# composewell/streamly-lz4

Hardware: AMD Instinct MI355X
Metric: GB/s uncompressed (compress+decompress), 64 KiB blocks, 1/2/4/8 GPU (higher is better)
Workload: dtype u8

## Files before the change

### streamly-lz4_amd/csrc/decode_par.hpp

```cpp
#pragma once

#include "decode_seq.hpp"

namespace lz4dev {

#define PAR_NODES 512
#ifndef PAR_ADAPT
#define PAR_ADAPT 1
#endif
#ifndef PAR_TAIL_ROUND
#define PAR_TAIL_ROUND 2
#endif
#ifndef PAR_ADAPT6
#define PAR_ADAPT6 416
#endif
#ifndef PAR_ADAPT10
#define PAR_ADAPT10 0
#endif
#define PAR_MAXNODES (PAR_ADAPT10 ? 640 : 512)
#ifndef PAR_SQ
#define PAR_SQ 3
#endif
#ifndef PAR_WIN
#define PAR_WIN 832
#endif
#ifndef PAR_RING
#define PAR_RING 5728
#endif
#ifndef PAR_HIST
#define PAR_HIST 2000
#endif
#ifndef PAR_BATCH_OUT
#define PAR_BATCH_OUT 2048
#endif
#ifndef PAR_FAR_WIDE
#define PAR_FAR_WIDE 0
#endif
#ifndef PAR_RANK
#define PAR_RANK 1
#endif
#ifndef PAR_PRIO
#define PAR_PRIO 0x33
#endif
#ifndef PAR_WAVES
#define PAR_WAVES 5
#endif

struct __attribute__((aligned(16))) ParLds {
    uint8_t win[PAR_WIN + 32];
    uint16_t jump[PAR_MAXNODES + 8];
    uint8_t ring[PAR_RING + 32];
};
#define PAR_END (2 * PAR_NODES)
#ifndef PAR_LDS_LIMIT
#define PAR_LDS_LIMIT 7680
#endif
static_assert(sizeof(ParLds) <= PAR_LDS_LIMIT, "ParLds above six 1280-byte LDS granules: 18 waves per CU instead of 20");
#define PAR_WIN_LANES (PAR_WIN / 16)
static_assert(PAR_WIN % 16 == 0 && PAR_WIN_LANES <= LZ4_WAVE, "the window is 16 bytes per lane");
static_assert(PAR_MAXNODES + 288 <= PAR_WIN + 32, "a plain sequence that starts at the last node, and the reads behind it, stay in win[]");
static_assert(PAR_HIST + 30 + PAR_BATCH_OUT + 32 <= PAR_RING, "a batch fits the ring right after a slide");

typedef uint64_t par_u64u __attribute__((aligned(1)));
typedef uint32_t par_u32u __attribute__((aligned(1)));
typedef uint16_t par_u16u __attribute__((aligned(1)));

typedef uint32_t par_v4 __attribute__((ext_vector_type(4)));
typedef par_v4 par_v4u __attribute__((aligned(1)));

__device__ __forceinline__ uint32_t lds_u32_any(const uint8_t *base4, uint32_t addr)
{
    const uint32_t *p = (const uint32_t *)(base4 + (addr & ~3u));
    return __builtin_amdgcn_alignbyte(p[1], p[0], addr & 3u);
}
__device__ __forceinline__ uint64_t lds_u64_any(const uint8_t *base4, uint32_t addr)
{
    const uint32_t *p = (const uint32_t *)(base4 + (addr & ~3u));
    const uint32_t d0 = p[0], d1 = p[1], d2 = p[2];
    const uint32_t sh = addr & 3u;
    return ((uint64_t)__builtin_amdgcn_alignbyte(d2, d1, sh) << 32) | __builtin_amdgcn_alignbyte(d1, d0, sh);
}

__device__ __forceinline__ int par_bperm(int v, int srcLane)
{
    return __builtin_amdgcn_ds_bpermute(srcLane << 2, v);
}

template <int D>
__device__ __forceinline__ int par_row_shr(int v)
{
    return __builtin_amdgcn_update_dpp(0, v, 0x110 | D, 0xf, 0xf, true);
}

__device__ __forceinline__ int par_scan_incl(int x)
{
    x += __builtin_amdgcn_update_dpp(0, x, 0x111, 0xf, 0xf, true);
    x += __builtin_amdgcn_update_dpp(0, x, 0x112, 0xf, 0xf, true);
    x += __builtin_amdgcn_update_dpp(0, x, 0x114, 0xf, 0xf, true);
    x += __builtin_amdgcn_update_dpp(0, x, 0x118, 0xf, 0xf, true);
    x += __builtin_amdgcn_update_dpp(0, x, 0x142, 0xa, 0xf, false);
    x += __builtin_amdgcn_update_dpp(0, x, 0x143, 0xc, 0xf, false);
    return x;
}

enum { PS_BATCHES, PS_SEQS, PS_ROUNDS, PS_MATCH_ITERS, PS_LIT_ITERS, PS_HANDOVERS, PS_SLIDES, PS_FULL, PS_FAR,
       PS_T_WINDOW, PS_T_SPEC, PS_T_CHAIN, PS_T_DECODE, PS_T_LIT, PS_T_NEED, PS_T_MATCH, PS_T_FLUSH, PS_T_SEQ, PS_COUNT };

template <bool STATS, bool DICT, bool TOL = false, bool LIST = false, bool PARTIAL = false>
__device__ int decode_block_par(const uint8_t *src, int srcLen, uint8_t *dst, int cap, const uint8_t *dict,
                                uint32_t dictLen, const uint8_t *bufLo, const uint8_t *bufHi, ParLds &L,
                                unsigned long long *stats, TolCtx *tol = nullptr, const uint8_t *list = nullptr,
                                int listLen = 0)
{
    int li = 0;
    int nodesPerLane = 8;
    uint32_t sc[PS_COUNT];
    uint32_t tmark = 0;
    if (STATS) {
#pragma unroll
        for (int i = 0; i < PS_COUNT; i++) sc[i] = 0;
        tmark = (uint32_t)__builtin_amdgcn_readfirstlane((int)(uint32_t)__builtin_amdgcn_s_memtime());
    }
    auto lap = [&](int which) {
        if (STATS) {
            const uint32_t now = (uint32_t)__builtin_amdgcn_readfirstlane((int)(uint32_t)__builtin_amdgcn_s_memtime());
            sc[which] += now - tmark;
            tmark = now;
        }
    };
    auto publish = [&]() {
        if (STATS && lane_id() == 0) {
#pragma unroll
            for (int i = 0; i < PS_COUNT; i++) atomicAdd(&stats[i], (unsigned long long)sc[i]);
        }
    };
    static_assert(!PARTIAL || (!DICT && !TOL), "the partial mode has no dictionary");
    if (cap < 128 || srcLen < 64) return decode_block_seq<TOL, PARTIAL>(src, srcLen, dst, cap, dict, dictLen, bufLo, bufHi, tol);
    if (!DICT) { dict = nullptr; dictLen = 0; }
    const uint8_t *dictEnd = DICT ? dict + dictLen : dst;
    const int dictLo = DICT ? -(int)min(dictLen, 65535u) : 0;

    int lane = lane_id();
    const int iend = srcLen;
    const uint32_t A = (uint32_t)((uintptr_t)dst & 15);
    int ip = 0, op = 0;
    int ringBase = 0;
    int flushed = 0;
    SeqState st;

    auto win_lane = [&]() -> int { return (PAR_WIN_LANES < LZ4_WAVE) ? min(lane, PAR_WIN_LANES - 1) : lane; };
    auto fetch_window = [&](uintptr_t base) -> uint4 {
        const uint8_t *q = (const uint8_t *)(base + 16u * (uint32_t)win_lane());
        if (q >= bufLo && q + 16 <= bufHi) {
            const par_v4 v = *as_global((const par_v4 *)q);
            return make_uint4(v.x, v.y, v.z, v.w);
        }
        uint32_t w[4] = {0, 0, 0, 0};
        for (int k = 0; k < 16; k++)
            if (q + k >= bufLo && q + k < bufHi) w[k >> 2] |= (uint32_t)as_global(q)[k] << (8 * (k & 3));
        return make_uint4(w[0], w[1], w[2], w[3]);
    };

#ifndef PAR_FLUSH
#define PAR_FLUSH 64
#endif
    const uint32_t AF = (uint32_t)((uintptr_t)dst & (PAR_FLUSH - 1));
    auto flush = [&](int upto, bool final) {
        wave_fence();
        int f = flushed;
        const int mis = (int)((AF + (uint32_t)f) & (PAR_FLUSH - 1));
        if (mis) {
            const int head = PAR_FLUSH - mis;
            if (upto - f >= head) {
                if (lane < head) dst[f + lane] = L.ring[f - ringBase + (int)A + lane];
                f += head;
            } else if (!final) {
                return;
            }
        }
        if (((AF + (uint32_t)f) & (PAR_FLUSH - 1)) == 0) {
            const int n16 = final ? (upto - f) >> 4 : ((upto - f) / PAR_FLUSH) * (PAR_FLUSH / 16);
            for (int c = lane; c < n16; c += LZ4_WAVE) {
                const uint4 v = *(const uint4 *)&L.ring[f - ringBase + (int)A + 16 * c];
                *(uint4 *)(dst + f + 16 * c) = v;
            }
            f += n16 << 4;
        }
        if (final) {
            for (int x = f + lane; x < upto; x += LZ4_WAVE) dst[x] = L.ring[x - ringBase + (int)A];
            f = upto;
        }
        flushed = f;
        wave_fence();
    };

    uintptr_t wbase = (uintptr_t)src & ~(uintptr_t)15;
    uint4 wnext = fetch_window(wbase);
    bool winStale = true;
    const uint8_t *jumpB = (const uint8_t *)L.jump;

    for (;;) {
        while (iend - ip >= 64 && cap - op >= 128) {
            lap(PS_T_FLUSH);

            const uint8_t *gp = src + ip;
            const uintptr_t abase = (uintptr_t)gp & ~(uintptr_t)15;
            const int wofs = (int)((uintptr_t)gp - abase);
            const int ipW0 = ip - wofs;
            const int iendW = iend - ipW0;
            const int inLim = min(iendW - 32, PAR_WIN);
            if (abase != wbase) { wbase = abase; wnext = fetch_window(abase); winStale = true; }
            if (winStale) {
                *(uint4 *)&L.win[16 * win_lane()] = wnext;
                winStale = false;
                wave_fence();
            }
            lap(PS_T_WINDOW);

            uint32_t c2, absorb;
            bool fromList = false;
            if (LIST && li < listLen) {
                fromList = true;
                absorb = 2u * (uint32_t)max(inLim, 0);
                const int k = li + lane;
                const uint32_t d = (k < listLen) ? (uint32_t)as_global(list)[k] : 0u;
                const uint64_t zm = __ballot(d == 0u);
                const int known = zm ? (int)__builtin_ctzll(zm) : LZ4_WAVE - 1;
                const int incl0 = par_scan_incl((int)d);
                c2 = (lane <= known) ? 2u * (uint32_t)(wofs + incl0 - (int)d) : absorb;
                c2 = min(c2, absorb);
            } else {
            auto parse_square = [&](auto NC) {
                constexpr int NL = decltype(NC)::value;
                static_assert(NL % 2 == 0 && NL * LZ4_WAVE <= PAR_MAXNODES, "pairs of nodes, table size");
                uint32_t J[NL];
                absorb = 2u * ((uint32_t)min(inLim, NL * LZ4_WAVE - 1) + 1u);
                {
                    typedef unsigned short par_h2 __attribute__((ext_vector_type(2)));
                    uint32_t w0, w1, w2;
                    if (NL == 8) {
                        const uint64_t lo = *(const uint64_t *)&L.win[8 * lane];
                        w0 = (uint32_t)lo; w1 = (uint32_t)(lo >> 32);
                        w2 = (uint32_t)__builtin_amdgcn_update_dpp(0, (int)w0, 0x130, 0xf, 0xf, false);
                    } else {
                        const uint32_t a = (uint32_t)(NL * lane);
                        const uint32_t *q = (const uint32_t *)&L.win[a & ~3u];
                        const uint32_t d0 = q[0], d1 = q[1], d2 = q[2], d3 = q[3];
                        const uint32_t sh = a & 3u;
                        w0 = __builtin_amdgcn_alignbyte(d1, d0, sh);
                        w1 = __builtin_amdgcn_alignbyte(d2, d1, sh);
                        w2 = __builtin_amdgcn_alignbyte(d3, d2, sh);
                    }
                    auto h2 = [](uint32_t x) { par_h2 r; __builtin_memcpy(&r, &x, 4); return r; };
                    auto u32 = [](par_h2 x) { uint32_t r; __builtin_memcpy(&r, &x, 4); return r; };
                    const par_h2 one = {1, 1}, lim = h2((absorb >> 1) * 0x00010001u);
                    const uint32_t base3 = ((uint32_t)(NL * lane) + 3u) * 0x00010001u + 0x00010000u;
                    uint32_t P[NL / 2];
#pragma unroll
                    for (int p = 0; p < NL / 2; p++) {
                        const uint32_t ws = (p < 2) ? w0 : ((p < 4) ? w1 : w2), wn = (p < 2) ? w1 : w2;
                        const par_h2 T = h2(__builtin_amdgcn_perm(0u, ws, (p & 1) ? 0x0c030c02u : 0x0c010c00u));
                        const par_h2 B = h2((p & 1) ? __builtin_amdgcn_perm(wn, ws, 0x0c040c03u) : __builtin_amdgcn_perm(0u, ws, 0x0c020c01u));
                        const par_h2 lit0 = T >> 4;
                        const par_h2 ext = (lit0 + one) >> 4;
                        const par_h2 term = ext * (B + one) + lit0;
                        const par_h2 mlx = ((T & (par_h2){15, 15}) + one) >> 4;
                        const par_h2 nxt = term + mlx + h2(base3 + 0x00020002u * (uint32_t)p);
                        P[p] = u32(__builtin_elementwise_min(nxt, lim) << 1);
                    }
                    uint32_t *tw = (uint32_t *)&L.jump[NL * lane];
#pragma unroll
                    for (int p = 0; p < NL / 2; p++) tw[p] = P[p];
                    if (lane == 0) L.jump[NL * LZ4_WAVE] = (uint16_t)(2 * NL * LZ4_WAVE);
#pragma unroll
                    for (int p = 0; p < NL / 2; p++) { J[2 * p] = P[p] & 0xffffu; J[2 * p + 1] = P[p] >> 16; }
                }
                wave_fence();
                lap(PS_T_SPEC);
#if PAR_PRIO
            if ((PAR_PRIO >> 0 & 3) != (PAR_PRIO >> 6 & 3)) __builtin_amdgcn_s_setprio(PAR_PRIO >> 0 & 3);
#endif

                c2 = (lane == 0) ? 2u * (uint32_t)wofs : absorb;
#pragma unroll
                for (int k = 0; k < PAR_SQ; k++) {
                    const int d = 1 << k;
                    const int cj = (int)*(const uint16_t *)(jumpB + c2);
#pragma unroll
                    for (int j = 0; j < NL; j++) J[j] = (uint32_t)*(const uint16_t *)(jumpB + J[j]);
                    int sh;
                    if (k == 0) sh = par_row_shr<1>(cj);
                    else if (k == 1) sh = par_row_shr<2>(cj);
                    else if (k == 2) sh = par_row_shr<4>(cj);
                    else sh = par_row_shr<8>(cj);
                    if (lane >= d && lane < 2 * d) c2 = (uint32_t)sh;
                    wave_fence();
                    uint32_t *tw = (uint32_t *)&L.jump[NL * lane];
#pragma unroll
                    for (int p = 0; p < NL / 2; p++) tw[p] = J[2 * p] | (J[2 * p + 1] << 16);
                    wave_fence();
                }
            };
#ifdef PAR_FORCE_NL
            parse_square(std::integral_constant<int, PAR_FORCE_NL>());
#elif PAR_ADAPT
            if (nodesPerLane == 6) parse_square(std::integral_constant<int, 6>());
#if PAR_ADAPT10
            else if (nodesPerLane == 10) parse_square(std::integral_constant<int, 10>());
#endif
            else
                parse_square(std::integral_constant<int, 8>());
#else
                parse_square(std::integral_constant<int, 8>());
#endif
            {
                constexpr int G = 1 << PAR_SQ;
#pragma unroll
                for (int g = 1; g < LZ4_WAVE / G; g++) {
                    int cj = (int)absorb;
                    if (lane >= G * (g - 1) && lane < G * g) cj = (int)*(const uint16_t *)(jumpB + c2);
                    int sh;
                    if (G == 1 && (g & 15)) sh = par_row_shr<1>(cj);
                    else if (G == 2 && (g & 7)) sh = par_row_shr<2>(cj);
                    else if (G == 4 && (g & 3)) sh = par_row_shr<4>(cj);
                    else if (G == 8 && (g & 1)) sh = par_row_shr<8>(cj);
#ifndef PAR_GROUP_BPERM
                    else if (G == 8 && (g == 2 || g == 6)) {
                        const auto r = __builtin_amdgcn_permlane16_swap((unsigned)cj, (unsigned)cj, false, false);
                        sh = __builtin_amdgcn_update_dpp(0, (int)r[0], 0x128 , 0xf, 0xf, false);
                    } else if (G == 8 && g == 4) {
                        const auto q = __builtin_amdgcn_permlane32_swap((unsigned)cj, (unsigned)cj, false, false);
                        const auto r = __builtin_amdgcn_permlane16_swap(q[0], q[0], false, false);
                        sh = __builtin_amdgcn_update_dpp(0, (int)r[1], 0x128 , 0xf, 0xf, false);
                    }
#endif
                    else sh = par_bperm(cj, (lane - G) & 63);
                    if (lane >= G * g && lane < G * g + G) c2 = (uint32_t)sh;
                }
            }
            }
            lap(PS_T_CHAIN);
#if PAR_PRIO
            if ((PAR_PRIO >> 2 & 3) != (PAR_PRIO >> 0 & 3)) __builtin_amdgcn_s_setprio(PAR_PRIO >> 2 & 3);
#endif

            const bool has = c2 < absorb;
            const uint32_t cc = has ? (c2 >> 1) : 0u;
            const uint32_t tb = lds_u32_any(L.win, cc);
            const uint32_t t = tb & 0xffu, b1 = (tb >> 8) & 0xffu;
            const bool is15 = (t >> 4) == 15u;
            const uint32_t lit = is15 ? 15u + b1 : (t >> 4);
            const uint32_t litStart = cc + 1u + (is15 ? 1u : 0u);
            const uint32_t offPos = litStart + lit;
            const uint32_t ob = lds_u32_any(L.win, offPos);
            const uint32_t off16 = ob & 0xffffu, b2 = (ob >> 16) & 0xffu;
            const bool mlx = (t & 15u) == 15u;
            const uint32_t ml = (t & 15u) + LZ4_MINMATCH + (mlx ? b2 : 0u);
            const uint32_t nxt = offPos + 2u + (mlx ? 1u : 0u);
            bool ok = has && !(is15 && b1 == 255u) && !(mlx && b2 == 255u) && (int)nxt <= inLim && off16 != 0;
            bool listBad = false;
            if (LIST && fromList) {
                const uint32_t prevNxt = (uint32_t)__builtin_amdgcn_update_dpp(0, (int)nxt, 0x138 , 0xf, 0xf, false);
                listBad = has && lane > 0 && prevNxt != cc;
                ok = ok && !listBad;
            }
            const int len = ok ? (int)(lit + ml) : 0;
            const int incl = par_scan_incl(len);
            const int outEnd = op + incl;
            const int outStart = outEnd - len;
            const int dpos = outStart + (int)lit;
            const int spos = dpos - (int)off16;
            ok = ok && incl <= PAR_BATCH_OUT && outEnd + 64 < cap &&
                 ((spos >= 0 && (spos >= ringBase || spos + (int)ml <= flushed)) ||
                  (DICT && spos >= dictLo && spos + (int)ml <= 0 && (!PAR_FAR_WIDE || ml >= 16u || spos + 16 <= 0)) ||
                  (TOL && spos < 0));
            const uint64_t okm = __ballot(ok);
            const int nseq = (~okm) ? (int)__builtin_ctzll(~okm) : LZ4_WAVE;
            if (LIST && fromList) {
                if (nseq < LZ4_WAVE && ((__ballot(listBad) >> nseq) & 1ull)) listLen = 0;
                li += nseq;
            }
            lap(PS_T_DECODE);
            if (STATS) { sc[PS_BATCHES]++; sc[PS_SEQS] += (unsigned)nseq; if (nseq == LZ4_WAVE) sc[PS_FULL]++; }
            if (nseq == 0) break;

            const bool act = lane < nseq;
            const int opNext = __builtin_amdgcn_readlane(outEnd, nseq - 1);
            const int ipNext = ipW0 + __builtin_amdgcn_readlane((int)nxt, nseq - 1);
            if (PAR_ADAPT && !fromList && nseq >= 16) {
                const int need = (ipNext - ip) * LZ4_WAVE;
                nodesPerLane = (need <= PAR_ADAPT6 * nseq) ? 6 : ((need <= 520 * nseq || !PAR_ADAPT10) ? 8 : 10);
            } else if (PAR_ADAPT && !fromList && nodesPerLane == 6 && !((__ballot(has) >> nseq) & 1ull)) {
                nodesPerLane = 8;
            }
            const uint32_t mdA = (uint32_t)(dpos - ringBase) + A;
            const bool ext = TOL && spos < 0;
            const bool nearSrc = spos >= ringBase && !ext;
            bool deferred = false;
            const bool w8 = ml >= 8 && off16 >= 8;
            const bool grp = w8 && (off16 >= 32 || off16 >= ml);
            const bool g16 = grp && ml >= 16;
            const bool g8 = grp && ml < 16;
            const bool g4 = ml < 8 && off16 >= ml;
            const bool fastc = g16 || g8 || g4;

            const uint64_t farm = __ballot(act && !nearSrc);
            if (TOL && farm) {
                if (act && !nearSrc && (ext || tol_tainted(tol, spos, spos + (int)ml))) {
                    deferred = true;
                    tol_taint(tol, dpos, dpos + (int)ml);
                }
                wave_fence();
            }
            const uint8_t *gsrc = (DICT && spos < 0) ? dictEnd + spos : dst + spos;
            const bool farMine = act && !nearSrc && !deferred;
            const uint32_t fstep = (ml >= 16) ? 16u : ((ml >= 8) ? 8u : 4u);
            const uint32_t flast = ml - fstep;
            par_v4 f0 = {0u, 0u, 0u, 0u}, f1 = {0u, 0u, 0u, 0u};
            uint64_t fa = 0, fb = 0;
            uint32_t fw0 = 0, fw1 = 0;
            if (farm) {
                if (STATS) sc[PS_FAR] += (unsigned)__builtin_popcountll(farm);
#if PAR_FAR_WIDE
                if (farMine) __builtin_memcpy(&f0, gsrc, 16);
                if (farMine && fstep == 16 && ml > 16u) __builtin_memcpy(&f1, gsrc + min(16u, flast), 16);
#else
                if (farMine && fstep == 16) {
                    __builtin_memcpy(&f0, gsrc, 16);
                    __builtin_memcpy(&f1, gsrc + min(16u, flast), 16);
                }
                if (farMine && fstep == 8) {
                    fa = *(const par_u64u *)(gsrc);
                    fb = *(const par_u64u *)(gsrc + flast);
                }
                if (farMine && fstep == 4) {
                    fw0 = *(const par_u32u *)(gsrc);
                    fw1 = *(const par_u32u *)(gsrc + flast);
                }
#endif
            }
            {
                const uintptr_t nb = (uintptr_t)(src + ipNext) & ~(uintptr_t)15;
                wbase = nb;
                wnext = fetch_window(nb);
            }

            uint64_t need = 0;
#if PAR_RANK
            {
                static_assert(16 * (PAR_BATCH_OUT / 64 + 1) <= 2 * PAR_NODES, "rank records fit the jump table");
                uint8_t *rk = (uint8_t *)L.jump;
                constexpr int NREC = PAR_BATCH_OUT / 64 + 1;
                {
                    uint32_t z = 0;
                    asm volatile("" : "+v"(z));
                    if (lane < NREC) *(uint4 *)&rk[16 * lane] = make_uint4(z, z, z, z);
                }
                wave_fence();
                if (act) {
                    const uint32_t rel = (uint32_t)(outStart - op);
                    atomicOr((uint32_t *)&rk[16u * (rel >> 6) + 4u * ((rel >> 5) & 1u)], 1u << (rel & 31u));
                }
                wave_fence();
                {
                    uint2 w = make_uint2(0u, 0u);
                    if (lane < NREC) w = *(const uint2 *)&rk[16 * lane];
                    const int cnt = (int)__builtin_popcount(w.x) + (int)__builtin_popcount(w.y);
                    const int pre = par_scan_incl(cnt) - cnt;
                    if (lane < NREC) *(uint32_t *)&rk[16 * lane + 8] = (uint32_t)pre;
                }
                wave_fence();
                const int srcHi = min(spos + (int)ml, outStart);
                if (act && nearSrc && srcHi > op && srcHi > spos) {
                    const uint32_t xlo = (uint32_t)(max(spos, op) - op), xhi = (uint32_t)(srcHi - 1 - op);
                    auto rank = [&](uint32_t x) -> int {
                        const uint4 r = *(const uint4 *)&rk[16u * (x >> 6)];
                        const uint32_t m = (2u << (x & 31u)) - 1u;
                        const bool hi = (x & 32u) != 0u;
                        return (int)r.z + (int)__builtin_popcount(r.x & (hi ? ~0u : m)) + (int)__builtin_popcount(r.y & (hi ? m : 0u)) - 1;
                    };
                    const int jlo = rank(xlo), jhi = rank(xhi);
                    const uint64_t upto = (jhi >= 63) ? ~0ull : ((1ull << (jhi + 1)) - 1ull);
                    need = upto & ~((1ull << jlo) - 1ull);
                    need &= ~(1ull << lane);
                }
                wave_fence();
            }
#else
            {
                const int srcHi = min(spos + (int)ml, outStart);
                const int xlo = max(spos, op), xhi = max(srcHi - 1, op);
                int jlo = 0, jhi = 0;
#pragma unroll
                for (int stp = 32; stp >= 1; stp >>= 1) {
                    const int c1 = jlo + stp, cb = jhi + stp;
                    const int v1 = par_bperm(outStart, c1 & 63), v2 = par_bperm(outStart, cb & 63);
                    if (c1 < nseq && v1 <= xlo) jlo = c1;
                    if (cb < nseq && v2 <= xhi) jhi = cb;
                }
                if (act && nearSrc && srcHi > op && srcHi > spos) {
                    const uint64_t upto = (jhi >= 63) ? ~0ull : ((1ull << (jhi + 1)) - 1ull);
                    need = upto & ~((1ull << jlo) - 1ull);
                    need &= ~(1ull << lane);
                }
            }
#endif
            {
                const uint32_t sA = litStart;
                const uint32_t dA = (uint32_t)(outStart - ringBase) + A;
                const uint32_t n = act ? lit : 0u;
                if (n > 16) {
                    const uint32_t last = n - 16;
                    for (uint32_t o = 0;; o += 16) {
                        const uint32_t oo = min(o, last);
                        *(par_v4u *)&L.ring[dA + oo] = *(const par_v4u *)&L.win[sA + oo];
                        if (o >= last) break;
                    }
                } else if (n > 8) {
                    if (n + ml >= 16) {
                        *(par_v4u *)&L.ring[dA] = *(const par_v4u *)&L.win[sA];
                    } else {
                        const uint64_t a = *(const par_u64u *)&L.win[sA], b = *(const par_u64u *)&L.win[sA + n - 8];
                        *(par_u64u *)&L.ring[dA] = a;
                        *(par_u64u *)&L.ring[dA + n - 8] = b;
                    }
                } else if (n > 0) {
                    const uint64_t v = lds_u64_any(L.win, sA);
                    if (n + ml >= 8) {
                        *(par_u64u *)&L.ring[dA] = v;
                    } else {
                        uint64_t w = v;
                        for (uint32_t q = 0; q < n; q++) { L.ring[dA + q] = (uint8_t)w; w >>= 8; }
                    }
                }
            }
            wave_fence();

            if (farm) {
#if PAR_FAR_WIDE
                if (fstep == 16 && ml <= 16u) f1 = f0;
                {
                    const uint32_t sh = ml - 8u;
                    const bool up = (sh & 4u) != 0u;
                    const uint32_t lo = up ? f0.y : f0.x, mid = up ? f0.z : f0.y, hi = up ? f0.w : f0.z;
                    fa = (uint64_t)f0.x | ((uint64_t)f0.y << 32);
                    fb = (uint64_t)__builtin_amdgcn_alignbyte(mid, lo, sh & 3u) | ((uint64_t)__builtin_amdgcn_alignbyte(hi, mid, sh & 3u) << 32);
                    fw0 = f0.x;
                    fw1 = __builtin_amdgcn_alignbyte(f0.y, f0.x, (ml - 4u) & 3u);
                }
#endif
                if (farMine && fstep == 16) {
                    *(par_v4u *)&L.ring[mdA] = f0;
                    *(par_v4u *)&L.ring[mdA + min(16u, flast)] = f1;
                }
                if (farMine && fstep == 8) {
                    *(par_u64u *)&L.ring[mdA] = fa;
                    *(par_u64u *)&L.ring[mdA + flast] = fb;
                }
                if (farMine && fstep == 4) {
                    *(par_u32u *)&L.ring[mdA] = fw0;
                    *(par_u32u *)&L.ring[mdA + flast] = fw1;
                }
                for (uint32_t base = 32; __ballot(farMine && base < ml); base += 32) {
                    par_v4 v0 = {0u, 0u, 0u, 0u}, v1 = {0u, 0u, 0u, 0u};
                    const bool on = farMine && base < ml;
                    const uint32_t o0 = min(base, flast), o1 = min(base + 16u, flast);
                    if (on) {
                        __builtin_memcpy(&v0, gsrc + o0, 16);
                        __builtin_memcpy(&v1, gsrc + o1, 16);
                    }
                    if (on) {
                        *(par_v4u *)&L.ring[mdA + o0] = v0;
                        *(par_v4u *)&L.ring[mdA + o1] = v1;
                    }
                }
            }

            lap(PS_T_NEED);
#if PAR_PRIO
            if ((PAR_PRIO >> 4 & 3) != (PAR_PRIO >> 2 & 3)) __builtin_amdgcn_s_setprio(PAR_PRIO >> 4 & 3);
#endif
            need &= ~farm;
            uint64_t done = ((nseq >= LZ4_WAVE) ? 0ull : (~0ull << nseq)) | farm;
            bool pending = act && nearSrc;
            const uint32_t msA = nearSrc ? (uint32_t)(spos - ringBase) + A : 0u;
            int roundNo = 0;
            while (~done) {
#if PAR_TAIL_ROUND
                if (!TOL && roundNo >= PAR_TAIL_ROUND) {
                    for (uint64_t sm = __ballot(pending); sm; sm &= sm - 1) {
                        if (STATS) sc[PS_MATCH_ITERS]++;
                        const int k = (int)__builtin_ctzll(sm);
                        const uint32_t kd = (uint32_t)__builtin_amdgcn_readlane((int)mdA, k);
                        const uint32_t ks = (uint32_t)__builtin_amdgcn_readlane((int)msA, k);
                        const uint32_t koff = (uint32_t)__builtin_amdgcn_readlane((int)off16, k);
                        const uint32_t kml = (uint32_t)__builtin_amdgcn_readlane((int)ml, k);
                        if (koff >= kml) {
                            if ((uint32_t)lane < kml) L.ring[kd + (uint32_t)lane] = L.ring[ks + (uint32_t)lane];
                            for (uint32_t j = (uint32_t)lane + LZ4_WAVE; j < kml; j += LZ4_WAVE) L.ring[kd + j] = L.ring[ks + j];
                        } else {
                            const float rcp = 1.0f / (float)koff;
                            for (uint32_t j = (uint32_t)lane; j < kml; j += LZ4_WAVE) {
                                const uint32_t q = (uint32_t)((float)j * rcp);
                                int rem = (int)j - (int)(q * koff);
                                if (rem < 0) rem += (int)koff; else if (rem >= (int)koff) rem -= (int)koff;
                                L.ring[kd + j] = L.ring[ks + (uint32_t)rem];
                            }
                        }
                        wave_fence();
                    }
                    pending = false;
                    break;
                }
                roundNo++;
#endif
                const bool ready = pending && ((need & ~done) == 0ull);
                bool mine = ready;
                if (TOL) {
                    const int srcHi = min(spos + (int)ml, dpos);
                    if (ready && srcHi > spos && tol_tainted(tol, spos, srcHi)) {
                        deferred = true;
                        mine = false;
                        tol_taint(tol, dpos, dpos + (int)ml);
                    }
                    wave_fence();
                }
                if (STATS) sc[PS_ROUNDS]++;
                for (uint32_t base = 0; __ballot(mine && fastc && base < ml); base += 32) {
                    if (STATS) sc[PS_MATCH_ITERS]++;
                    const bool on = mine && fastc && base < ml;
                    const uint32_t cs = g16 ? 16u : (g8 ? 8u : 4u);
                    const uint32_t lastc = ml - cs;
                    const uint32_t o0 = g16 ? min(base, lastc) : 0u;
                    const uint32_t o1 = g16 ? min(base + 16u, lastc) : lastc;
                    par_v4 v0 = {0u, 0u, 0u, 0u}, v1 = {0u, 0u, 0u, 0u};
                    uint64_t na = 0, nc = 0;
                    uint32_t nw0 = 0, nw1 = 0;
                    if (on) v0 = *(const par_v4u *)&L.ring[msA + o0];
                    if (on && g16 && ml > 16u) v1 = *(const par_v4u *)&L.ring[msA + o1];
                    if (g16 && ml <= 16u) v1 = v0;
                    {
                        const uint32_t sh = ml - 8u;
                        const bool up = (sh & 4u) != 0u;
                        const uint32_t lo = up ? v0.y : v0.x, mid = up ? v0.z : v0.y, hi = up ? v0.w : v0.z;
                        na = (uint64_t)v0.x | ((uint64_t)v0.y << 32);
                        nc = (uint64_t)__builtin_amdgcn_alignbyte(mid, lo, sh & 3u) | ((uint64_t)__builtin_amdgcn_alignbyte(hi, mid, sh & 3u) << 32);
                        nw0 = v0.x;
                        nw1 = __builtin_amdgcn_alignbyte(v0.y, v0.x, (ml - 4u) & 3u);
                    }
                    if (on && g16) {
                        *(par_v4u *)&L.ring[mdA + o0] = v0;
                        *(par_v4u *)&L.ring[mdA + o1] = v1;
                    }
                    if (on && g8) {
                        *(par_u64u *)&L.ring[mdA] = na;
                        *(par_u64u *)&L.ring[mdA + o1] = nc;
                    }
                    if (on && g4) {
                        *(par_u32u *)&L.ring[mdA] = nw0;
                        *(par_u32u *)&L.ring[mdA + o1] = nw1;
                    }
                    wave_fence();
                }
                for (uint64_t sm = __ballot(mine && !fastc); sm; sm &= sm - 1) {
                    if (STATS) sc[PS_MATCH_ITERS]++;
                    const int k = (int)__builtin_ctzll(sm);
                    const uint32_t kd = (uint32_t)__builtin_amdgcn_readlane((int)mdA, k);
                    const uint32_t ks = (uint32_t)__builtin_amdgcn_readlane((int)msA, k);
                    const uint32_t koff = (uint32_t)__builtin_amdgcn_readlane((int)off16, k);
                    const uint32_t kml = (uint32_t)__builtin_amdgcn_readlane((int)ml, k);
                    const float rcp = 1.0f / (float)koff;
                    for (uint32_t j = (uint32_t)lane; j < kml; j += LZ4_WAVE) {
                        const uint32_t q = (uint32_t)((float)j * rcp);
                        int rem = (int)j - (int)(q * koff);
                        if (rem < 0) rem += (int)koff; else if (rem >= (int)koff) rem -= (int)koff;
                        L.ring[kd + j] = L.ring[ks + (uint32_t)rem];
                    }
                    wave_fence();
                }
                pending = pending && !ready;
                done |= __ballot(ready);
            }
            wave_fence();
            if (TOL) {
                const uint64_t dm = __ballot(deferred);
                if (dm) {
                    const uint32_t rank = __builtin_amdgcn_mbcnt_hi((uint32_t)(dm >> 32), __builtin_amdgcn_mbcnt_lo((uint32_t)dm, 0u));
                    const uint32_t base = tol->count;
                    if (deferred && base + rank < tol->cap) tol->list[base + rank] = tol_entry(dpos, spos, ml);
                    wave_fence();
                    if (lane == 0) tol->count = base + (uint32_t)__builtin_popcountll(dm);
                    wave_fence();
                }
            }
            lap(PS_T_MATCH);
#if PAR_PRIO
            if ((PAR_PRIO >> 6 & 3) != (PAR_PRIO >> 4 & 3)) __builtin_amdgcn_s_setprio(PAR_PRIO >> 6 & 3);
#endif

            op = opNext;
            ip = ipNext;
            *(uint4 *)&L.win[16 * win_lane()] = wnext;
            wave_fence();
            flush(op, false);
            if (op - ringBase + (int)A + PAR_BATCH_OUT + 32 > PAR_RING) {
                if (STATS) sc[PS_SLIDES]++;
                const int newBase = (op - PAR_HIST) & ~15;
                const int delta = newBase - ringBase;
                const int n16 = (op - newBase + (int)A + 15) >> 4;
                constexpr int PAR_SLIDE = (PAR_HIST + 45 + 16 * LZ4_WAVE - 1) / (16 * LZ4_WAVE);
                {
                    uint4 v[PAR_SLIDE];
#pragma unroll
                    for (int i = 0; i < PAR_SLIDE; i++) {
                        const int k = lane + i * LZ4_WAVE;
                        v[i] = (k < n16) ? *(const uint4 *)&L.ring[delta + 16 * k] : make_uint4(0u, 0u, 0u, 0u);
                    }
                    wave_fence();
#pragma unroll
                    for (int i = 0; i < PAR_SLIDE; i++) {
                        const int k = lane + i * LZ4_WAVE;
                        if (k < n16) *(uint4 *)&L.ring[16 * k] = v[i];
                    }
                }
                ringBase = newBase;
                wave_fence();
            }
        }

        flush(op, true);
        st.ip = ip; st.op = op; st.fast = true;
        const bool tail = (iend - ip < 64 || cap - op < 128);
        if (STATS && !tail) sc[PS_HANDOVERS]++;
        lap(PS_T_FLUSH);
        int r = decode_seq_dispatch<TOL, PARTIAL>(st, tail ? 0 : 1, src, srcLen, dst, cap, dict, dictLen, bufLo, bufHi, tol);
        if (r == SEQ_CONTINUE && (!st.fast || iend - st.ip < 64 || cap - st.op < 128))
            r = decode_seq_dispatch<TOL, PARTIAL>(st, 0, src, srcLen, dst, cap, dict, dictLen, bufLo, bufHi, tol);
        lap(PS_T_SEQ);
        r = uni(r);
        if (r != SEQ_CONTINUE) { publish(); return r; }
        ip = uni(st.ip); op = uni(st.op);
        if (LIST) li += 1;
        asm volatile("v_mbcnt_lo_u32_b32 %0, -1, 0\n\tv_mbcnt_hi_u32_b32 %0, -1, %0" : "=v"(lane));
        wbase = (uintptr_t)(src + ip) & ~(uintptr_t)15;
        wnext = fetch_window(wbase);
        winStale = true;
        wave_fence();
        ringBase = (op > PAR_HIST) ? ((op - PAR_HIST) & ~15) : 0;
        flushed = op;
        for (int x = ringBase + lane; x < op; x += LZ4_WAVE) L.ring[x - ringBase + (int)A] = dst[x];
        wave_fence();
        lap(PS_T_SEQ);
    }
}

}
```

### streamly-lz4_amd/csrc/kernels/decode_par_cu.inc

```
#ifdef PAR_WAVES_MAX
#define PAR_OCC __attribute__((amdgpu_flat_work_group_size(64, 64), amdgpu_waves_per_eu(PAR_WAVES, PAR_WAVES_MAX)))
#else
#define PAR_OCC __launch_bounds__(64, PAR_WAVES)
#endif
template <bool STATS>
__global__ PAR_OCC void k_decode_par(DecodeArgs a, unsigned long long *stats)
{
    __shared__ ParLds lds;
    const int blk = (int)blockIdx.x;
    const uint8_t *data = nullptr;
    int compLen = 0, cap = 0;
    int r = read_block_header(a, blk, data, compLen, cap);
    if (r == 0)
        r = decode_block_par<STATS, false>(data, compLen, a.out + a.outOff[blk], cap, nullptr, 0, a.framed,
                                    a.framed + a.framedLen, lds, stats);
    if (lane_id() == 0) a.result[blk] = r;
}

void launch_decode_par(const DecodeArgs &a, unsigned long long *stats, hipStream_t s)
{
    if (a.nBlocks <= 0) return;
    if (stats)
        hipLaunchKernelGGL(k_decode_par<true>, dim3((unsigned)a.nBlocks), dim3(64), 0, s, a, stats);
    else
        hipLaunchKernelGGL(k_decode_par<false>, dim3((unsigned)a.nBlocks), dim3(64), 0, s, a, stats);
    launch_link_stat(a, s);
}

__global__ PAR_OCC void k_decode_par_redo(DecodeArgs a)
{
    __shared__ ParLds lds;
    const int blk = (int)blockIdx.x;
    if (uni(a.result[blk]) != CU_REDO) return;
    const uint8_t *data = nullptr;
    int compLen = 0, cap = 0;
    int r = read_block_header(a, blk, data, compLen, cap);
    if (r == 0)
        r = decode_block_par<false, false, false, true>(data, compLen, a.out + a.outOff[blk], cap, nullptr, 0, a.framed,
                                                        a.framed + a.framedLen, lds, nullptr, nullptr, nullptr, 0);
    if (lane_id() == 0) a.result[blk] = r;
}

__global__ __launch_bounds__(CU_THREADS) void k_decode_cu(DecodeArgs a)
{
    __shared__ __attribute__((aligned(16))) uint8_t lds[CU_LDS_BYTES];
    const int blk = (int)blockIdx.x;
    const uint8_t *data = nullptr;
    int compLen = 0, cap = 0;
    int r = uni(read_block_header(a, blk, data, compLen, cap));
    if (r == 0 && a.cuBail && (int64_t)uni(compLen) * 16 > (int64_t)uni(cap) * 15) r = CU_REDO;
    else if (r == 0)
        r = decode_block_cu<false>(data, uni(compLen), a.out + a.outOff[blk], uni(cap), nullptr, 0, a.framed, a.framed + a.framedLen, lds,
                                   a.cuDbg ? a.cuDbg + 16 * (size_t)blk : nullptr, a.cuBail != 0);
    if (threadIdx.x == 0) a.result[blk] = r;
    const bool prevFinal = blk == 0 && a.lookBack > 0 && a.cu.res && uni(a.result[-1]) >= 65536;
    if (a.cu.res && (blk > 0 || prevFinal) && r == CU_REDO && !(a.cuBail && (int64_t)uni(compLen) * 16 > (int64_t)uni(cap) * 15)) {
        __syncthreads();
        const uint8_t *dict = prevFinal ? a.out + a.outOff[-1] + (size_t)uni(a.result[-1]) - 65536u : a.run.zeroPage;
        const int r2 = decode_block_cu<true>(data, uni(compLen), a.out + a.outOff[blk], uni(cap), dict, 65536u, a.framed,
                                            a.framed + a.framedLen, lds, nullptr, false, 0);
        if (threadIdx.x == 0) {
            a.cu.res[blk] = r2;
            if (r2 < 0 || (r2 < 65536 && blk + 1 < a.nBlocks)) atomicAdd(&a.cu.flags[1], 1u);
        }
    }
}

__global__ __launch_bounds__(CU_THREADS) void k_decode_cu_linked(DecodeArgs a)
{
    __shared__ __attribute__((aligned(16))) uint8_t lds[CU_LDS_BYTES];
    const int blk = (int)blockIdx.x;
    if (uni(a.result[blk]) >= 0) return;
    const uint8_t *dict = nullptr;
    if (blk == 0) {
        const bool prevFinal = a.lookBack > 0 && uni(a.result[-1]) >= 65536;
        if (prevFinal && uni(a.cu.res[0]) >= 65536) return;
        if (!prevFinal || a.cu.pass != 1) { if (threadIdx.x == 0) atomicAdd(&a.cu.flags[1], 1u); return; }
        dict = a.out + a.outOff[-1] + (size_t)uni(a.result[-1]) - 65536u;
    } else {
        if (a.cu.pass > 2 && uni(a.cu.flags[2 + blk - 1]) == 0u) return;
        dict = a.cu.pass == 1 ? a.run.zeroPage : a.cu.snap + (size_t)(blk - 1) * 65536u;
    }
    const uint8_t *data = nullptr;
    int compLen = 0, cap = 0;
    int r = uni(read_block_header(a, blk, data, compLen, cap));
    if (r == 0)
        r = decode_block_cu<true>(data, uni(compLen), a.out + a.outOff[blk], uni(cap), dict, 65536u, a.framed, a.framed + a.framedLen, lds, nullptr, false,
                                  (blk > 0 && a.cu.pass > 1 && uni(a.cu.res[blk]) >= 65536) ? uni(a.cu.res[blk]) : 0);
    if (threadIdx.x == 0) {
        a.cu.res[blk] = r;
        if (r < 0 || (r < 65536 && blk + 1 < a.nBlocks)) atomicAdd(&a.cu.flags[1], 1u);
    }
}

__global__ __launch_bounds__(1024) void k_cu_tails(DecodeArgs a)
{
    const int blk = (int)blockIdx.x;
    if (blk + 1 >= a.nBlocks) return;
    const int32_t r = a.result[blk] >= 0 ? a.result[blk] : a.cu.res[blk];
    __shared__ uint32_t diff;
    if (threadIdx.x == 0) diff = 0u;
    __syncthreads();
    uint32_t d = 0u;
    if (r >= 65536) {
        const uint8_t *tail = a.out + a.outOff[blk] + (size_t)r - 65536u;
        uint8_t *snap = a.cu.snap + (size_t)blk * 65536u;
        for (uint32_t i = threadIdx.x * 16u; i < 65536u; i += 1024u * 16u) {
            const par_v4 v = *(const par_v4u *)(tail + i), o = *(const par_v4 *)(snap + i);
            d |= (v.x ^ o.x) | (v.y ^ o.y) | (v.z ^ o.z) | (v.w ^ o.w);
            *(par_v4 *)(snap + i) = v;
        }
    }
    if (d) atomicOr(&diff, 1u);
    __syncthreads();
    if (threadIdx.x == 0) {
        if (r < 65536 && a.result[blk + 1] < 0) atomicAdd(&a.cu.flags[1], 1u);
        const uint32_t ch = (diff != 0u || a.cu.pass == 1) ? 1u : 0u;
        a.cu.flags[2 + blk] = ch;
        if (ch) atomicAdd(&a.cu.flags[0], 1u);
    }
}

__global__ __launch_bounds__(256) void k_cu_publish(DecodeArgs a)
{
    const int blk = (int)(blockIdx.x * 256u + threadIdx.x);
    if (blk < a.nBlocks && a.result[blk] < 0) a.result[blk] = a.cu.res[blk];
}

void launch_cu_linked(const DecodeArgs &a, bool decode, hipStream_t s)
{
    if (a.nBlocks <= 0) return;
    hipMemsetAsync(a.cu.flags, 0, 4, s);
    if (decode) hipLaunchKernelGGL(k_decode_cu_linked, dim3((unsigned)a.nBlocks), dim3(CU_THREADS), 0, s, a);
    hipLaunchKernelGGL(k_cu_tails, dim3((unsigned)a.nBlocks), dim3(1024), 0, s, a);
}

void launch_cu_publish(const DecodeArgs &a, hipStream_t s)
{
    hipLaunchKernelGGL(k_cu_publish, dim3((unsigned)((a.nBlocks + 255) / 256)), dim3(256), 0, s, a);
}

void launch_decode_cu(const DecodeArgs &a, hipStream_t s)
{
    if (a.nBlocks <= 0) return;
    hipLaunchKernelGGL(k_decode_cu, dim3((unsigned)a.nBlocks), dim3(CU_THREADS), 0, s, a);
    hipLaunchKernelGGL(k_decode_par_redo, dim3((unsigned)a.nBlocks), dim3(64), 0, s, a);
    launch_link_stat(a, s);
}
```

Measured before the change: 1085.

## Overlay jump table onto ring tail and shrink LDS to raise decode occupancy

Moves the jump table and rank records into the unused tail of the output ring and shrinks the ring and history window, so the per-wave LDS footprint fits five granules. The main decode kernels then request six waves per EU instead of five. The aim is more concurrent waves per CU to hide memory latency. It also replaces the byte-by-byte edge window fetch with one clamped vector load plus byte shifts, and adds uniformity hints around the sequential handover. The risks are a shorter history, which can force more slides or far-match fallbacks, and register pressure from the tighter occupancy target causing spills.

```diff
diff --git a/streamly-lz4_amd/csrc/decode_par.hpp b/streamly-lz4_amd/csrc/decode_par.hpp
--- a/streamly-lz4_amd/csrc/decode_par.hpp
+++ b/streamly-lz4_amd/csrc/decode_par.hpp
@@ -25,10 +25,10 @@
 #define PAR_WIN 832
 #endif
 #ifndef PAR_RING
-#define PAR_RING 5728
+#define PAR_RING 5504
 #endif
 #ifndef PAR_HIST
-#define PAR_HIST 2000
+#define PAR_HIST 1776
 #endif
 #ifndef PAR_BATCH_OUT
 #define PAR_BATCH_OUT 2048
@@ -45,17 +45,26 @@
 #ifndef PAR_WAVES
 #define PAR_WAVES 5
 #endif
-
+#ifndef PAR_WAVES_MAIN
+#define PAR_WAVES_MAIN (PAR_WAVES > 6 ? PAR_WAVES : 6)
+#endif
+
+#define PAR_JUMP_BYTES (2 * (PAR_MAXNODES + 8))
+#define PAR_JUMP_OFS ((PAR_RING + 32 - PAR_JUMP_BYTES) & ~15)
 struct __attribute__((aligned(16))) ParLds {
     uint8_t win[PAR_WIN + 32];
-    uint16_t jump[PAR_MAXNODES + 8];
     uint8_t ring[PAR_RING + 32];
+    __device__ __forceinline__ uint16_t *jump() { return (uint16_t *)&ring[PAR_JUMP_OFS]; }
 };
 #define PAR_END (2 * PAR_NODES)
 #ifndef PAR_LDS_LIMIT
-#define PAR_LDS_LIMIT 7680
-#endif
-static_assert(sizeof(ParLds) <= PAR_LDS_LIMIT, "ParLds above six 1280-byte LDS granules: 18 waves per CU instead of 20");
+#define PAR_LDS_LIMIT 6400
+#endif
+static_assert(sizeof(ParLds) <= PAR_LDS_LIMIT, "ParLds above five 1280-byte LDS granules: 20 waves per CU or fewer instead of 24");
+static_assert((PAR_WIN + 32) % 16 == 0 && PAR_JUMP_OFS % 16 == 0, "the table and its 16-byte rank records are aligned");
+static_assert(PAR_JUMP_OFS + PAR_JUMP_BYTES <= PAR_RING + 32, "the table lies inside ring[]");
+static_assert(PAR_JUMP_BYTES <= PAR_BATCH_OUT + 32 && PAR_JUMP_OFS >= ((PAR_RING - PAR_BATCH_OUT - 32 + 15) & ~15),
+              "the table overlays ring bytes that hold no output when a batch is parsed (the no-slide bound)");
 #define PAR_WIN_LANES (PAR_WIN / 16)
 static_assert(PAR_WIN % 16 == 0 && PAR_WIN_LANES <= LZ4_WAVE, "the window is 16 bytes per lane");
 static_assert(PAR_MAXNODES + 288 <= PAR_WIN + 32, "a plain sequence that starts at the last node, and the reads behind it, stay in win[]");
@@ -103,6 +112,27 @@
     return x;
 }
 
+__device__ __forceinline__ uint4 par_fetch_window_edge(const uint8_t *q, const uint8_t *bufLo, const uint8_t *bufHi)
+{
+    uint32_t E[8] = {0u, 0u, 0u, 0u, 0u, 0u, 0u, 0u};
+    uint32_t m = 0;
+    if (q + 16 > bufLo && q < bufHi) {
+        const uint8_t *qc = (q < bufLo) ? bufLo : bufHi - 16;
+        par_v4 v;
+        __builtin_memcpy(&v, as_global(qc), 16);
+        const bool below = q < bufLo;
+        const uint32_t d = (uint32_t)(below ? bufLo - q : q - qc);
+        m = below ? 16u - d : d;
+        E[0] = below ? 0u : v.x; E[1] = below ? 0u : v.y; E[2] = below ? 0u : v.z; E[3] = below ? 0u : v.w;
+        E[4] = below ? v.x : 0u; E[5] = below ? v.y : 0u; E[6] = below ? v.z : 0u; E[7] = below ? v.w : 0u;
+    }
+    if (m & 8u) { for (int i = 0; i < 6; i++) E[i] = E[i + 2]; }
+    if (m & 4u) { for (int i = 0; i < 5; i++) E[i] = E[i + 1]; }
+    uint32_t w[4];
+    for (int i = 0; i < 4; i++) w[i] = __builtin_amdgcn_alignbyte(E[i + 1], E[i], m & 3u);
+    return make_uint4(w[0], w[1], w[2], w[3]);
+}
+
 enum { PS_BATCHES, PS_SEQS, PS_ROUNDS, PS_MATCH_ITERS, PS_LIT_ITERS, PS_HANDOVERS, PS_SLIDES, PS_FULL, PS_FAR,
        PS_T_WINDOW, PS_T_SPEC, PS_T_CHAIN, PS_T_DECODE, PS_T_LIT, PS_T_NEED, PS_T_MATCH, PS_T_FLUSH, PS_T_SEQ, PS_COUNT };
 
@@ -140,7 +170,8 @@
     const uint8_t *dictEnd = DICT ? dict + dictLen : dst;
     const int dictLo = DICT ? -(int)min(dictLen, 65535u) : 0;
 
-    int lane = lane_id();
+    int lane;
+    asm volatile("v_mbcnt_lo_u32_b32 %0, -1, 0\n\tv_mbcnt_hi_u32_b32 %0, -1, %0" : "=v"(lane));
     const int iend = srcLen;
     const uint32_t A = (uint32_t)((uintptr_t)dst & 15);
     int ip = 0, op = 0;
@@ -151,14 +182,11 @@
     auto win_lane = [&]() -> int { return (PAR_WIN_LANES < LZ4_WAVE) ? min(lane, PAR_WIN_LANES - 1) : lane; };
     auto fetch_window = [&](uintptr_t base) -> uint4 {
         const uint8_t *q = (const uint8_t *)(base + 16u * (uint32_t)win_lane());
-        if (q >= bufLo && q + 16 <= bufHi) {
+        if (__builtin_expect(q >= bufLo && q + 16 <= bufHi, 1)) {
             const par_v4 v = *as_global((const par_v4 *)q);
             return make_uint4(v.x, v.y, v.z, v.w);
         }
-        uint32_t w[4] = {0, 0, 0, 0};
-        for (int k = 0; k < 16; k++)
-            if (q + k >= bufLo && q + k < bufHi) w[k >> 2] |= (uint32_t)as_global(q)[k] << (8 * (k & 3));
-        return make_uint4(w[0], w[1], w[2], w[3]);
+        return par_fetch_window_edge(q, bufLo, bufHi);
     };
 
 #ifndef PAR_FLUSH
@@ -197,7 +225,7 @@
     uintptr_t wbase = (uintptr_t)src & ~(uintptr_t)15;
     uint4 wnext = fetch_window(wbase);
     bool winStale = true;
-    const uint8_t *jumpB = (const uint8_t *)L.jump;
+    const uint8_t *jumpB = (const uint8_t *)L.jump();
 
     for (;;) {
         while (iend - ip >= 64 && cap - op >= 128) {
@@ -268,10 +296,10 @@
                         const par_h2 nxt = term + mlx + h2(base3 + 0x00020002u * (uint32_t)p);
                         P[p] = u32(__builtin_elementwise_min(nxt, lim) << 1);
                     }
-                    uint32_t *tw = (uint32_t *)&L.jump[NL * lane];
+                    uint32_t *tw = (uint32_t *)&L.jump()[NL * lane];
 #pragma unroll
                     for (int p = 0; p < NL / 2; p++) tw[p] = P[p];
-                    if (lane == 0) L.jump[NL * LZ4_WAVE] = (uint16_t)(2 * NL * LZ4_WAVE);
+                    if (lane == 0) L.jump()[NL * LZ4_WAVE] = (uint16_t)(2 * NL * LZ4_WAVE);
 #pragma unroll
                     for (int p = 0; p < NL / 2; p++) { J[2 * p] = P[p] & 0xffffu; J[2 * p + 1] = P[p] >> 16; }
                 }
@@ -295,7 +323,7 @@
                     else sh = par_row_shr<8>(cj);
                     if (lane >= d && lane < 2 * d) c2 = (uint32_t)sh;
                     wave_fence();
-                    uint32_t *tw = (uint32_t *)&L.jump[NL * lane];
+                    uint32_t *tw = (uint32_t *)&L.jump()[NL * lane];
 #pragma unroll
                     for (int p = 0; p < NL / 2; p++) tw[p] = J[2 * p] | (J[2 * p + 1] << 16);
                     wave_fence();
@@ -449,7 +477,7 @@
 #if PAR_RANK
             {
                 static_assert(16 * (PAR_BATCH_OUT / 64 + 1) <= 2 * PAR_NODES, "rank records fit the jump table");
-                uint8_t *rk = (uint8_t *)L.jump;
+                uint8_t *rk = (uint8_t *)L.jump();
                 constexpr int NREC = PAR_BATCH_OUT / 64 + 1;
                 {
                     uint32_t z = 0;
@@ -733,8 +761,10 @@
         const bool tail = (iend - ip < 64 || cap - op < 128);
         if (STATS && !tail) sc[PS_HANDOVERS]++;
         lap(PS_T_FLUSH);
+        if (!DICT && !TOL && !PARTIAL) asm volatile("" : "=v"(lane), "=v"(wnext.x), "=v"(wnext.y), "=v"(wnext.z), "=v"(wnext.w));
         int r = decode_seq_dispatch<TOL, PARTIAL>(st, tail ? 0 : 1, src, srcLen, dst, cap, dict, dictLen, bufLo, bufHi, tol);
-        if (r == SEQ_CONTINUE && (!st.fast || iend - st.ip < 64 || cap - st.op < 128))
+        r = uni(r);
+        if (r == SEQ_CONTINUE && (!uni((int)st.fast) || iend - uni(st.ip) < 64 || cap - uni(st.op) < 128))
             r = decode_seq_dispatch<TOL, PARTIAL>(st, 0, src, srcLen, dst, cap, dict, dictLen, bufLo, bufHi, tol);
         lap(PS_T_SEQ);
         r = uni(r);
diff --git a/streamly-lz4_amd/csrc/kernels/decode_par_cu.inc b/streamly-lz4_amd/csrc/kernels/decode_par_cu.inc
--- a/streamly-lz4_amd/csrc/kernels/decode_par_cu.inc
+++ b/streamly-lz4_amd/csrc/kernels/decode_par_cu.inc
@@ -3,8 +3,13 @@
 #else
 #define PAR_OCC __launch_bounds__(64, PAR_WAVES)
 #endif
+#ifdef PAR_WAVES_MAX
+#define PAR_OCC_MAIN __attribute__((amdgpu_flat_work_group_size(64, 64), amdgpu_waves_per_eu(PAR_WAVES_MAIN, (PAR_WAVES_MAX > PAR_WAVES_MAIN ? PAR_WAVES_MAX : PAR_WAVES_MAIN))))
+#else
+#define PAR_OCC_MAIN __launch_bounds__(64, PAR_WAVES_MAIN)
+#endif
 template <bool STATS>
-__global__ PAR_OCC void k_decode_par(DecodeArgs a, unsigned long long *stats)
+__global__ PAR_OCC_MAIN void k_decode_par(DecodeArgs a, unsigned long long *stats)
 {
     __shared__ ParLds lds;
     const int blk = (int)blockIdx.x;
@@ -27,7 +32,7 @@
     launch_link_stat(a, s);
 }
 
-__global__ PAR_OCC void k_decode_par_redo(DecodeArgs a)
+__global__ PAR_OCC_MAIN void k_decode_par_redo(DecodeArgs a)
 {
     __shared__ ParLds lds;
     const int blk = (int)blockIdx.x;
```

After: 1153 (median of 6 runs). +6.3%, better.
